# chinhau5/parallel_eda

Hardware: AMD Instinct MI355X
Metric: place+route wall-clock to feasibility (s/flow; bitcoin_miner-scale synthetic on stratixiv-like fabric) (lower is better)
Workload: dtype fp32; 1 GPU; model=bitcoin_miner, arch=bitcoin_stratixiv, grid=280x200, W=300, rr_nodes=15745036, rr_edges=87277236, blocks=37632, nets=35616, conns=110426, global_batch=110426, seq_len=0, final_overused=0, wirelength=4914127

## Files before the change

csrc/hip/place_kernel.hip:

```cpp
#include "pnr_hip.h"

namespace pnrh {

struct PlaceDev {
  const int32_t* net_blk_ptr;
  const int32_t* net_blks;
  const int32_t* blk_net_ptr;
  const int32_t* blk_nets;
  const int8_t* blk_type;
  const int8_t* tile_btype;
  const int32_t* type_cols;
  const int32_t* type_col_ptr;
  const uint8_t* fixed;
  const float* net_q;
  const int32_t* net_sink_ptr;
  const float* conn_crit;
  const float* delay_mat;
  int32_t* bx;
  int32_t* by;
  int32_t* bslot;
  int32_t* grid;
  float* net_cost;
  float* net_tcost;
  int32_t num_blocks, num_nets, gx, gy, cap, nx, ny, io_cap;
  int32_t rx0, rx1;
  const int32_t* macro_of;
  const int32_t* macro_ptr;
  const int32_t* macro_blk;
};

struct MovesDev {
  int32_t* mv_blk;
  int32_t* mv_to;
  int32_t* mv_other;
  float* mv_dbb;
  float* mv_dtd;
  uint8_t* mv_flags;
  int32_t* net_claim;
  int32_t* loc_claim;
  int32_t* counters;
  int32_t n_moves;
};

struct Sched {
  float T; int rlim; float timing_tradeoff, inv_bb_norm, inv_td_norm;
  uint32_t seed, batch;
};

#define PROP_WAVES 4

__device__ __forceinline__ int move_index() {
  return blockIdx.x * PROP_WAVES + (threadIdx.x >> 6);
}

__device__ __forceinline__ uint32_t rng_hash(uint32_t a, uint32_t b, uint32_t c) {
  uint32_t h = a * 0x9E3779B9u ^ b * 0x85EBCA6Bu ^ c * 0xC2B2AE35u;
  h ^= h >> 16; h *= 0x7FEB352Du; h ^= h >> 15; h *= 0x846CA68Bu; h ^= h >> 16;
  return h;
}

__device__ __forceinline__ bool is_io_loc(const PlaceDev& p, int x, int y) {
  return x == 0 || x == p.gx - 1 || y == 0 || y == p.gy - 1;
}
__device__ __forceinline__ int cap_at(const PlaceDev& p, int x, int y) {
  bool io = is_io_loc(p, x, y);
  if (!io && x >= 1 && x <= p.nx && y >= 1 && y <= p.ny) return 1;
  if (io && ((x >= 1 && x <= p.nx) != (y >= 1 && y <= p.ny))) return p.io_cap;
  return 0;
}

struct SwapPos {
  int32_t b1; int x1, y1; int32_t b2; int x2, y2;
  __device__ __forceinline__ void operator()(
      const PlaceDev&, int32_t b, int& x, int& y) const {
    if (b == b1) { x = x1; y = y1; }
    else if (b == b2) { x = x2; y = y2; }
  }
};
struct MacroPos {
  int mid, ddx, ddy;
  __device__ __forceinline__ void operator()(
      const PlaceDev& p, int32_t b, int& x, int& y) const {
    if (p.macro_of[b] == mid) { x += ddx; y += ddy; }
  }
};

template <class Pos> __device__ __forceinline__
float net_bb_cost(const PlaceDev& p, int n, const Pos& pos) {
  int xmin = 1 << 28, xmax = -1, ymin = 1 << 28, ymax = -1;
  int32_t e0 = p.net_blk_ptr[n], e1 = p.net_blk_ptr[n + 1];
  for (int32_t e = e0; e < e1; ++e) {
    int32_t b = p.net_blks[e];
    int x = p.bx[b], y = p.by[b];
    pos(p, b, x, y);
    xmin = min(xmin, x); xmax = max(xmax, x);
    ymin = min(ymin, y); ymax = max(ymax, y);
  }
  return p.net_q[n] * ((xmax - xmin + 1) + (ymax - ymin + 1));
}

template <class Pos> __device__ __forceinline__
float net_td_cost(const PlaceDev& p, int n, const Pos& pos) {
  if (p.delay_mat == nullptr) return 0.0f;
  int32_t e0 = p.net_blk_ptr[n], e1 = p.net_blk_ptr[n + 1];
  int32_t drv = p.net_blks[e0];
  int dx0 = p.bx[drv], dy0 = p.by[drv];
  pos(p, drv, dx0, dy0);
  float t = 0.0f;
  int32_t c0 = p.net_sink_ptr[n];
  for (int32_t e = e0 + 1; e < e1; ++e) {
    int32_t b = p.net_blks[e];
    int x = p.bx[b], y = p.by[b];
    pos(p, b, x, y);
    int dx = abs(x - dx0), dy = abs(y - dy0);
    t += p.conn_crit[c0 + (e - e0 - 1)] * p.delay_mat[dx * p.gy + dy];
  }
  return t;
}

__device__ __forceinline__ float wave_sum_f32(float v) {
  for (int off = 32; off; off >>= 1) v += __shfl_xor(v, off);
  return v;
}

__device__ __forceinline__
bool blk_has_net(const PlaceDev& p, int32_t b, int32_t n) {
  int32_t lo = p.blk_net_ptr[b], hi = p.blk_net_ptr[b + 1];
  while (lo < hi) {
    int32_t mid2 = (lo + hi) >> 1;
    if (p.blk_nets[mid2] < n) lo = mid2 + 1; else hi = mid2;
  }
  return lo < p.blk_net_ptr[b + 1] && p.blk_nets[lo] == n;
}

template <class F> __device__ __forceinline__
void for_blk_nets(const PlaceDev& p, int32_t b, F f) {
  for (int32_t k = p.blk_net_ptr[b] + (threadIdx.x & 63);
       k < p.blk_net_ptr[b + 1]; k += 64)
    f(p.blk_nets[k]);
}
template <class F> __device__ __forceinline__
void for_macro_nets(const PlaceDev& p, int32_t mm0, int32_t mm1, F f) {
  for (int32_t j = mm0; j < mm1; ++j)
    for_blk_nets(p, p.macro_blk[j], [&](int32_t n) { f(j, n); });
}

struct MinClaims {
  int32_t* net; int32_t* loc; int32_t mine;
  __device__ __forceinline__ void take_net(int n) const { atomicMin(&net[n], mine); }
  __device__ __forceinline__ void take_loc(int t) const { atomicMin(&loc[t], mine); }
  __device__ __forceinline__ bool holds_net(int n) const { return net[n] == mine; }
  __device__ __forceinline__ bool holds_loc(int t) const { return loc[t] == mine; }
};
struct EpochClaims {
  unsigned long long* net; unsigned long long* loc; unsigned long long mine;
  __device__ __forceinline__ void take_net(int n) const { atomicMax(&net[n], mine); }
  __device__ __forceinline__ void take_loc(int t) const { atomicMax(&loc[t], mine); }
  __device__ __forceinline__ bool holds_net(int n) const { return net[n] == mine; }
  __device__ __forceinline__ bool holds_loc(int t) const { return loc[t] == mine; }
};

__device__ __forceinline__ unsigned long long claim_key(uint32_t batch, int i) {
  return ((unsigned long long)batch << 32) | (0xFFFFFFFFu - (uint32_t)i);
}

__device__ __forceinline__
int propose_select(const PlaceDev& p, int rlim, uint32_t seed, uint32_t batch,
                   int i, int& x1o, int& y1o, int& slot1o) {
  uint32_t r0 = rng_hash(seed ^ 0x5BD1E995u, batch, i);
  int32_t blk = r0 % p.num_blocks;
  if (p.fixed && p.fixed[blk]) return -1;
  if (p.rx0 >= 0 && (p.bx[blk] < p.rx0 || p.bx[blk] > p.rx1))
    return -1;
  bool io = p.blk_type[blk] == 0;
  int x0 = p.bx[blk], y0 = p.by[blk];
  int x1 = -1, y1 = -1, slot1 = 0;
  int bt = p.blk_type[blk];
  if (p.tile_btype && bt >= 2 && p.type_cols) {
    int c0 = p.type_col_ptr[bt - 2], c1 = p.type_col_ptr[bt - 1];
    int lo = c0, hi = c1;
    while (lo < hi) { int m = (lo + hi) >> 1;
                      if (p.type_cols[m] < x0 - rlim) lo = m + 1; else hi = m; }
    int lo2 = lo, hi2 = c1;
    while (lo2 < hi2) { int m = (lo2 + hi2) >> 1;
                        if (p.type_cols[m] <= x0 + rlim) lo2 = m + 1; else hi2 = m; }
    int ncol = lo2 - lo;
    if (ncol > 0) {
      int ylo = max(1, y0 - rlim), yhi = min(p.ny, y0 + rlim);
      for (int att = 0; att < 8; ++att) {
        uint32_t r1 = rng_hash(seed, batch, i * 131 + 7 * att + 1);
        uint32_t r2 = rng_hash(seed, batch, i * 131 + 7 * att + 2);
        int tx = p.type_cols[lo + (int)(r1 % ncol)];
        if (p.rx0 >= 0 && (tx < p.rx0 || tx > p.rx1)) continue;
        int ty = ylo + (int)(r2 % (yhi - ylo + 1));
        if (tx == x0 && ty == y0) continue;
        x1 = tx; y1 = ty; slot1 = 0;
        break;
      }
    }
  } else {
    for (int att = 0; att < 8; ++att) {
      uint32_t r1 = rng_hash(seed, batch, i * 131 + 7 * att + 1);
      uint32_t r2 = rng_hash(seed, batch, i * 131 + 7 * att + 2);
      int tx = x0 + (int)(r1 % (2 * rlim + 1)) - rlim;
      int ty = y0 + (int)(r2 % (2 * rlim + 1)) - rlim;
      if (tx < 0 || tx >= p.gx || ty < 0 || ty >= p.gy) continue;
      if (p.rx0 >= 0 && (tx < p.rx0 || tx > p.rx1)) continue;
      if (p.tile_btype) {
        if (p.tile_btype[tx * p.gy + ty] != p.blk_type[blk]) continue;
      } else if (is_io_loc(p, tx, ty) != io) continue;
      int c = cap_at(p, tx, ty);
      if (c <= 0) continue;
      if (tx == x0 && ty == y0) continue;
      x1 = tx; y1 = ty;
      slot1 = (int)(rng_hash(seed, batch, i * 131 + 7 * att + 3) % c);
      break;
    }
  }
  if (x1 < 0) return -1;
  x1o = x1; y1o = y1; slot1o = slot1;
  return blk;
}

__device__ __forceinline__
bool macro_shift_ok(const PlaceDev& p, const MacroPos& ms, int32_t mm0,
                    int32_t mm1) {
  for (int32_t j = mm0; j < mm1; ++j) {
    int32_t b = p.macro_blk[j];
    int sx = p.bx[b], sy = p.by[b];
    int tx = sx + ms.ddx, ty = sy + ms.ddy;
    if (p.fixed && p.fixed[b]) return false;
    if (tx < 0 || tx >= p.gx || ty < 0 || ty >= p.gy) return false;
    if (p.rx0 >= 0 && (tx < p.rx0 || tx > p.rx1 ||
                       sx < p.rx0 || sx > p.rx1)) return false;
    if (p.tile_btype
            ? (p.tile_btype[tx * p.gy + ty] != p.blk_type[b])
            : (is_io_loc(p, tx, ty) != (p.blk_type[b] == 0))) return false;
    if (cap_at(p, tx, ty) != 1) return false;
    int32_t occ = p.grid[((int64_t)tx * p.gy + ty) * p.cap];
    if (occ >= 0 && p.macro_of[occ] != ms.mid) return false;
  }
  return true;
}

template <class Pos> __device__ __forceinline__
void add_net_delta(const PlaceDev& p, int32_t n, const Pos& pos,
                   float timing_tradeoff, float& dbb, float& dtd) {
  dbb += net_bb_cost(p, n, pos) - p.net_cost[n];
  if (timing_tradeoff > 0.0f)
    dtd += net_td_cost(p, n, pos) - p.net_tcost[n];
}

__device__ __forceinline__
bool metropolis(const Sched& s, int i, float& dbb, float& dtd) {
  dbb = wave_sum_f32(dbb);
  dtd = wave_sum_f32(dtd);
  float delta = (1.0f - s.timing_tradeoff) * dbb * s.inv_bb_norm +
                s.timing_tradeoff * dtd * s.inv_td_norm;
  if (delta <= 0.0f) return true;
  if (s.T <= 0.0f) return false;
  float u = (rng_hash(s.seed, s.batch, i * 131 + 5) & 0xFFFFFF) *
            (1.0f / 16777216.0f);
  return u < __expf(-delta / s.T);
}

__device__ __forceinline__
void record_move(const MovesDev& m, int32_t* mv_from, int i, int32_t blk,
                 int32_t to, int32_t other, float dbb, float dtd,
                 int32_t from) {
  atomicAdd(&m.counters[1], 1);
  m.mv_blk[i] = blk;
  m.mv_to[i] = to;
  m.mv_other[i] = other;
  m.mv_dbb[i] = dbb;
  m.mv_dtd[i] = dtd;
  m.mv_flags[i] = 1;
  mv_from[i] = from;
}

template <class Claims> __device__ __forceinline__
void propose_move(const PlaceDev& p, const MovesDev& m, const Claims& c,
                  int32_t* mv_from, int i, const Sched& s) {
  const int lane = threadIdx.x & 63;
  int sel = -1, sx1 = -1, sy1 = -1, sslot = 0;
  if (lane == 0) {
    m.mv_flags[i] = 0;
    sel = propose_select(p, s.rlim, s.seed, s.batch, i, sx1, sy1, sslot);
  }
  sel = __shfl(sel, 0);
  if (sel < 0) return;
  const int x1 = __shfl(sx1, 0);
  const int y1 = __shfl(sy1, 0);
  const int slot1 = __shfl(sslot, 0);
  const int32_t blk = sel;
  const int x0 = p.bx[blk], y0 = p.by[blk];
  const int mid = p.macro_of ? p.macro_of[blk] : -1;
  float dbb = 0.0f, dtd = 0.0f;
  if (mid >= 0) {
    const MacroPos ms{mid, x1 - x0, y1 - y0};
    const int32_t mm0 = p.macro_ptr[mid], mm1 = p.macro_ptr[mid + 1];
    if (mm1 - mm0 > 16) return;
    int ok = 0;
    if (lane == 0) {
      ok = macro_shift_ok(p, ms, mm0, mm1);
      if (ok) atomicAdd(&m.counters[0], 1);
    }
    ok = __shfl(ok, 0);
    if (!ok) return;
    for_macro_nets(p, mm0, mm1, [&](int32_t j, int32_t n) {
      bool dup = false;
      for (int32_t j2 = mm0; j2 < j && !dup; ++j2)
        dup = blk_has_net(p, p.macro_blk[j2], n);
      if (!dup) add_net_delta(p, n, ms, s.timing_tradeoff, dbb, dtd);
    });
    if (!metropolis(s, i, dbb, dtd)) return;
    if (lane == 0)
      record_move(m, mv_from, i, blk,
                  ((ms.ddx + 4096) << 13) | (ms.ddy + 4096), -2 - mid, dbb,
                  dtd, x0 * p.gy + y0);
    for_macro_nets(p, mm0, mm1, [&](int32_t, int32_t n) { c.take_net(n); });
    for (int32_t j = mm0 + lane; j < mm1; j += 64) {
      int32_t b = p.macro_blk[j];
      c.take_loc(p.bx[b] * p.gy + p.by[b]);
      c.take_loc((p.bx[b] + ms.ddx) * p.gy + p.by[b] + ms.ddy);
    }
    return;
  }
  int32_t other = p.grid[((int64_t)x1 * p.gy + y1) * p.cap + slot1];
  if (other == blk) return;
  if (other >= 0 && p.fixed && p.fixed[other]) return;
  if (other >= 0 && p.macro_of && p.macro_of[other] >= 0)
    return;
  if (lane == 0) atomicAdd(&m.counters[0], 1);
  const SwapPos sw{blk, x1, y1, other, other >= 0 ? x0 : -1000,
                   other >= 0 ? y0 : -1000};
  for_blk_nets(p, blk, [&](int32_t n) {
    add_net_delta(p, n, sw, s.timing_tradeoff, dbb, dtd);
  });
  if (other >= 0)
    for_blk_nets(p, other, [&](int32_t n) {
      if (!blk_has_net(p, blk, n))
        add_net_delta(p, n, sw, s.timing_tradeoff, dbb, dtd);
    });
  if (!metropolis(s, i, dbb, dtd)) return;
  if (lane == 0) {
    record_move(m, mv_from, i, blk, (x1 * p.gy + y1) * p.cap + slot1, other,
                dbb, dtd, x0 * p.gy + y0);
    c.take_loc(x0 * p.gy + y0);
    c.take_loc(x1 * p.gy + y1);
  }
  auto take = [&](int32_t n) { c.take_net(n); };
  for_blk_nets(p, blk, take);
  if (other >= 0) for_blk_nets(p, other, take);
}

struct Move {
  int32_t blk, other, to;
  __device__ __forceinline__ Move(const MovesDev& m, int i)
      : blk(m.mv_blk[i]), other(m.mv_other[i]), to(m.mv_to[i]) {}
  __device__ __forceinline__ bool is_macro() const { return other <= -2; }
  __device__ __forceinline__ MacroPos macro() const {
    return MacroPos{-2 - other, (to >> 13) - 4096, (to & 0x1FFF) - 4096};
  }
};

template <class Claims> __device__ __forceinline__
bool resolve_move(const PlaceDev& p, const MovesDev& m, const Claims& c,
                  const int32_t* mv_from, int i, const Move& mv) {
  const int lane = threadIdx.x & 63;
  bool bad = false;
  if (mv.is_macro()) {
    const MacroPos ms = mv.macro();
    const int32_t mm0 = p.macro_ptr[ms.mid], mm1 = p.macro_ptr[ms.mid + 1];
    for (int32_t j = mm0 + lane; j < mm1; j += 64) {
      int32_t b = p.macro_blk[j];
      int sx = p.bx[b], sy = p.by[b];
      int tx = sx + ms.ddx, ty = sy + ms.ddy;
      if (tx < 0 || tx >= p.gx || ty < 0 || ty >= p.gy) bad = true;
      else if (!c.holds_loc(sx * p.gy + sy) ||
               !c.holds_loc(tx * p.gy + ty)) bad = true;
    }
    for_macro_nets(p, mm0, mm1, [&](int32_t, int32_t n) {
      if (!c.holds_net(n)) bad = true;
    });
  } else {
    int x1 = mv.to / p.cap / p.gy, y1 = (mv.to / p.cap) % p.gy;
    if (lane == 0 && (!c.holds_loc(mv_from[i]) ||
                      !c.holds_loc(x1 * p.gy + y1))) bad = true;
    auto lost = [&](int32_t n) { if (!c.holds_net(n)) bad = true; };
    for_blk_nets(p, mv.blk, lost);
    if (mv.other >= 0) for_blk_nets(p, mv.other, lost);
  }
  const bool win = !__any(bad);
  if (lane == 0) {
    if (!win) { m.mv_flags[i] = 0; atomicAdd(&m.counters[3], 1); }
    else { m.mv_flags[i] = 2; atomicAdd(&m.counters[2], 1); }
  }
  return win;
}

template <class Pos> __device__ __forceinline__
void refresh_net(const PlaceDev& p, int32_t n, const Pos& pos,
                 float timing_tradeoff) {
  p.net_cost[n] = net_bb_cost(p, n, pos);
  if (timing_tradeoff > 0.0f) p.net_tcost[n] = net_td_cost(p, n, pos);
}

__device__ __forceinline__
void apply_move(const PlaceDev& p, const MovesDev& m, int i, const Move& mv,
                float timing_tradeoff, double* cost_acc ) {
  const int lane = threadIdx.x & 63;
  if (mv.is_macro()) {
    const MacroPos ms = mv.macro();
    const int32_t mm0 = p.macro_ptr[ms.mid], mm1 = p.macro_ptr[ms.mid + 1];
    for_macro_nets(p, mm0, mm1, [&](int32_t, int32_t n) {
      refresh_net(p, n, ms, timing_tradeoff);
    });
    if (lane == 0) {
      for (int32_t j = mm0; j < mm1; ++j) {
        int32_t b = p.macro_blk[j];
        p.grid[((int64_t)p.bx[b] * p.gy + p.by[b]) * p.cap + p.bslot[b]] = -1;
      }
      for (int32_t j = mm0; j < mm1; ++j) {
        int32_t b = p.macro_blk[j];
        int tx = p.bx[b] + ms.ddx, ty = p.by[b] + ms.ddy;
        p.grid[((int64_t)tx * p.gy + ty) * p.cap] = b;
        p.bx[b] = tx; p.by[b] = ty; p.bslot[b] = 0;
      }
    }
  } else {
    const int32_t blk = mv.blk, other = mv.other;
    int slot1 = mv.to % p.cap;
    int x1 = mv.to / p.cap / p.gy, y1 = (mv.to / p.cap) % p.gy;
    int x0 = p.bx[blk], y0 = p.by[blk], s0 = p.bslot[blk];
    const SwapPos sw{blk, x1, y1, other, other >= 0 ? x0 : -1000,
                     other >= 0 ? y0 : -1000};
    auto refresh = [&](int32_t n) { refresh_net(p, n, sw, timing_tradeoff); };
    for_blk_nets(p, blk, refresh);
    if (other >= 0) for_blk_nets(p, other, refresh);
    if (lane == 0) {
      p.grid[((int64_t)x0 * p.gy + y0) * p.cap + s0] = other >= 0 ? other : -1;
      p.grid[((int64_t)x1 * p.gy + y1) * p.cap + slot1] = blk;
      p.bx[blk] = x1; p.by[blk] = y1; p.bslot[blk] = slot1;
      if (other >= 0) { p.bx[other] = x0; p.by[other] = y0; p.bslot[other] = s0; }
    }
  }
  if (lane == 0) {
    unsafeAtomicAdd(&cost_acc[0], (double)m.mv_dbb[i]);
    unsafeAtomicAdd(&cost_acc[1], (double)m.mv_dtd[i]);
  }
}

__global__ void place_reset_claims_kernel(int32_t* net_claim, int32_t nn,
                                          int32_t* loc_claim, int32_t nl) {
  int i = blockIdx.x * blockDim.x + threadIdx.x;
  int total = max(nn, nl);
  for (; i < total; i += gridDim.x * blockDim.x) {
    if (i < nn) net_claim[i] = 0x7FFFFFFF;
    if (i < nl) loc_claim[i] = 0x7FFFFFFF;
  }
}

__launch_bounds__(64 * PROP_WAVES, 2)
__global__ void place_propose_kernel(PlaceDev p, MovesDev m, int32_t* mv_from,
                                     Sched s) {
  const int i = move_index();
  if (i >= m.n_moves) return;
  propose_move(p, m, MinClaims{m.net_claim, m.loc_claim, i}, mv_from, i, s);
}

__launch_bounds__(64 * PROP_WAVES, 2)
__global__ void place_resolve_kernel(PlaceDev p, MovesDev m,
                                     const int32_t* mv_from) {
  const int i = move_index();
  if (i >= m.n_moves || m.mv_flags[i] != 1) return;
  resolve_move(p, m, MinClaims{m.net_claim, m.loc_claim, i}, mv_from, i,
               Move(m, i));
}

__launch_bounds__(64 * PROP_WAVES, 2)
__global__ void place_apply_kernel(PlaceDev p, MovesDev m,
                                   float timing_tradeoff, double* cost_acc) {
  const int i = move_index();
  if (i >= m.n_moves || m.mv_flags[i] != 2) return;
  apply_move(p, m, i, Move(m, i), timing_tradeoff, cost_acc);
}

struct RunDev {
  int32_t* mv_from;
  unsigned long long* net_claim;
  unsigned long long* loc_claim;
  int32_t* ctrl;
};

__launch_bounds__(64 * PROP_WAVES, 2)
__global__ void place_propose_run_kernel(PlaceDev p, MovesDev m, RunDev r,
                                         Sched s) {
  if (r.ctrl[0]) return;
  const int i = move_index();
  if (i >= m.n_moves) return;
  const EpochClaims c{r.net_claim, r.loc_claim, claim_key(s.batch, i)};
  propose_move(p, m, c, r.mv_from, i, s);
}

__device__ __forceinline__
void commit_move(const PlaceDev& p, const MovesDev& m, const RunDev& r,
                 float timing_tradeoff, double* cost_acc, uint32_t batch) {
  const int i = move_index();
  if (i >= m.n_moves || m.mv_flags[i] != 1) return;
  const Move mv(m, i);
  const EpochClaims c{r.net_claim, r.loc_claim, claim_key(batch, i)};
  if (resolve_move(p, m, c, r.mv_from, i, mv))
    apply_move(p, m, i, mv, timing_tradeoff, cost_acc);
}

__launch_bounds__(64 * PROP_WAVES, 2)
__global__ void place_commit_kernel(PlaceDev p, MovesDev m, RunDev r,
                                    float timing_tradeoff, double* cost_acc,
                                    uint32_t batch, int check,
                                    int32_t target_moves) {
  if (r.ctrl[0]) return;
  commit_move(p, m, r, timing_tradeoff, cost_acc, batch);
  if (!check) return;
  asm volatile("s_waitcnt vmcnt(0)" ::: "memory");
  __syncthreads();
  if (threadIdx.x != 0) return;
  __threadfence();
  asm volatile("s_waitcnt vmcnt(0)" ::: "memory");
  int ticket = __hip_atomic_fetch_add(&r.ctrl[2], 1, __ATOMIC_RELAXED,
                                      __HIP_MEMORY_SCOPE_AGENT);
  if (ticket != (int)gridDim.x - 1) return;
  __threadfence();
  int att = __hip_atomic_load(&m.counters[0], __ATOMIC_RELAXED,
                              __HIP_MEMORY_SCOPE_AGENT);
  int acc = __hip_atomic_load(&m.counters[1], __ATOMIC_RELAXED,
                              __HIP_MEMORY_SCOPE_AGENT);
  int win = __hip_atomic_load(&m.counters[2], __ATOMIC_RELAXED,
                              __HIP_MEMORY_SCOPE_AGENT);
  r.ctrl[1] += 4;
  if (win + (att - acc) >= target_moves) r.ctrl[0] = 1;
  __hip_atomic_store(&r.ctrl[2], 0, __ATOMIC_RELAXED,
                     __HIP_MEMORY_SCOPE_AGENT);
}

__global__ void place_refresh_costs_kernel(PlaceDev p, float timing_tradeoff,
                                           double* out ) {
  int n = blockIdx.x * blockDim.x + threadIdx.x;
  for (; n < p.num_nets; n += gridDim.x * blockDim.x) {
    const SwapPos as_is{-1, 0, 0, -1, 0, 0};
    float c = net_bb_cost(p, n, as_is);
    p.net_cost[n] = c;
    unsafeAtomicAdd(&out[0], (double)c);
    float t = timing_tradeoff > 0.0f ? net_td_cost(p, n, as_is) : 0.0f;
    p.net_tcost[n] = t;
    unsafeAtomicAdd(&out[1], (double)t);
  }
}

}

using namespace pnrh;

extern "C" {

struct PlaceLaunchArgs {
  const int32_t* net_blk_ptr; const int32_t* net_blks;
  const int32_t* blk_net_ptr; const int32_t* blk_nets;
  const int8_t* blk_type; const int8_t* tile_btype;
  const int32_t* type_cols; const int32_t* type_col_ptr;
  const uint8_t* fixed;
  const float* net_q;
  const int32_t* net_sink_ptr; const float* conn_crit; const float* delay_mat;
  int32_t* bx; int32_t* by; int32_t* bslot; int32_t* grid;
  float* net_cost; float* net_tcost;
  int32_t num_blocks, num_nets, gx, gy, cap, nx, ny, io_cap;
  int32_t rx0, rx1;
  const int32_t* macro_of; const int32_t* macro_ptr;
  const int32_t* macro_blk;
  int32_t* mv_blk; int32_t* mv_to; int32_t* mv_other;
  float* mv_dbb; float* mv_dtd; uint8_t* mv_flags;
  int32_t* net_claim; int32_t* loc_claim; int32_t* counters;
  int32_t n_moves;
  float T; int32_t rlim; float timing_tradeoff;
  float inv_bb_norm, inv_td_norm;
  uint32_t seed, batch;
  double* cost_acc;
  int32_t* mv_from;
  unsigned long long* net_claim64; unsigned long long* loc_claim64;
  int32_t* run_ctrl;
};

static void unpack(const PlaceLaunchArgs* a, PlaceDev& p, MovesDev& m) {
  p.net_blk_ptr = a->net_blk_ptr; p.net_blks = a->net_blks;
  p.blk_net_ptr = a->blk_net_ptr; p.blk_nets = a->blk_nets;
  p.blk_type = a->blk_type; p.tile_btype = a->tile_btype;
  p.type_cols = a->type_cols; p.type_col_ptr = a->type_col_ptr;
  p.fixed = a->fixed;
  p.net_q = a->net_q;
  p.net_sink_ptr = a->net_sink_ptr; p.conn_crit = a->conn_crit;
  p.delay_mat = a->delay_mat;
  p.bx = a->bx; p.by = a->by; p.bslot = a->bslot; p.grid = a->grid;
  p.net_cost = a->net_cost; p.net_tcost = a->net_tcost;
  p.num_blocks = a->num_blocks; p.num_nets = a->num_nets;
  p.gx = a->gx; p.gy = a->gy; p.cap = a->cap;
  p.nx = a->nx; p.ny = a->ny; p.io_cap = a->io_cap;
  p.rx0 = a->rx0; p.rx1 = a->rx1;
  p.macro_of = a->macro_of; p.macro_ptr = a->macro_ptr;
  p.macro_blk = a->macro_blk;
  m.mv_blk = a->mv_blk; m.mv_to = a->mv_to; m.mv_other = a->mv_other;
  m.mv_dbb = a->mv_dbb; m.mv_dtd = a->mv_dtd; m.mv_flags = a->mv_flags;
  m.net_claim = a->net_claim; m.loc_claim = a->loc_claim;
  m.counters = a->counters; m.n_moves = a->n_moves;
}

static Sched sched(const PlaceLaunchArgs* a, uint32_t batch) {
  return Sched{a->T, a->rlim, a->timing_tradeoff, a->inv_bb_norm,
               a->inv_td_norm, a->seed, batch};
}

int pnr_place_batch(const PlaceLaunchArgs* a, void* stream) {
  if (!a->mv_from || !a->net_claim || !a->loc_claim)
    return (int)hipErrorInvalidValue;
  PlaceDev p; MovesDev m;
  unpack(a, p, m);
  hipStream_t s = (hipStream_t)stream;
  int rg = (max(max(a->num_nets, a->gx * a->gy), a->n_moves) + 255) / 256;
  rg = rg < 2048 ? rg : 2048;
  hipLaunchKernelGGL(place_reset_claims_kernel, dim3(rg), dim3(256), 0, s,
                     m.net_claim, p.num_nets, m.loc_claim, p.gx * p.gy);
  int mg = (m.n_moves + PROP_WAVES - 1) / PROP_WAVES;
  hipLaunchKernelGGL(place_propose_kernel, dim3(mg), dim3(64 * PROP_WAVES),
                     0, s, p, m, a->mv_from, sched(a, a->batch));
  hipLaunchKernelGGL(place_resolve_kernel, dim3(mg), dim3(64 * PROP_WAVES),
                     0, s, p, m, (const int32_t*)a->mv_from);
  hipLaunchKernelGGL(place_apply_kernel, dim3(mg), dim3(64 * PROP_WAVES),
                     0, s, p, m, a->timing_tradeoff, a->cost_acc);
  return (int)hipGetLastError();
}

int pnr_place_run(const PlaceLaunchArgs* a, uint32_t first_batch,
                  int32_t target_moves, int32_t n_batches, void* stream) {
  if (n_batches < 0 || (n_batches & 3) || first_batch == 0 ||
      !a->mv_from || !a->net_claim64 || !a->loc_claim64 || !a->run_ctrl)
    return (int)hipErrorInvalidValue;
  PlaceDev p; MovesDev m;
  unpack(a, p, m);
  RunDev r;
  r.mv_from = a->mv_from;
  r.net_claim = a->net_claim64; r.loc_claim = a->loc_claim64;
  r.ctrl = a->run_ctrl;
  hipStream_t s = (hipStream_t)stream;
  int mg = (m.n_moves + PROP_WAVES - 1) / PROP_WAVES;
  for (int32_t k = 0; k < n_batches; ++k) {
    const uint32_t batch = first_batch + (uint32_t)k;
    hipLaunchKernelGGL(place_propose_run_kernel, dim3(mg),
                       dim3(64 * PROP_WAVES), 0, s, p, m, r, sched(a, batch));
    hipLaunchKernelGGL(place_commit_kernel, dim3(mg), dim3(64 * PROP_WAVES),
                       0, s, p, m, r, a->timing_tradeoff, a->cost_acc, batch,
                       (int)(((k + 1) & 3) == 0), target_moves);
  }
  return (int)hipGetLastError();
}

int pnr_place_refresh(const PlaceLaunchArgs* a, void* stream) {
  PlaceDev p; MovesDev m;
  unpack(a, p, m);
  hipStream_t s = (hipStream_t)stream;
  hipLaunchKernelGGL(place_refresh_costs_kernel, dim3(1024), dim3(256), 0, s,
                     p, a->timing_tradeoff, a->cost_acc);
  return (int)hipGetLastError();
}

int64_t pnr_place_args_sizeof() { return (int64_t)sizeof(PlaceLaunchArgs); }

}
```

parallel_eda_amd/place/gpu_placer.py:

```python
import ctypes as ct
import math

import numpy as np

from ..arch.archdef import ArchDef
from ..ops import hip_api
from .placer import Placement, analytic_delay_matrix


class PlaceLaunchArgs(ct.Structure):
    _fields_ = [
        ("net_blk_ptr", ct.c_void_p), ("net_blks", ct.c_void_p),
        ("blk_net_ptr", ct.c_void_p), ("blk_nets", ct.c_void_p),
        ("blk_type", ct.c_void_p), ("tile_btype", ct.c_void_p),
        ("type_cols", ct.c_void_p), ("type_col_ptr", ct.c_void_p),
        ("fixed", ct.c_void_p),
        ("net_q", ct.c_void_p),
        ("net_sink_ptr", ct.c_void_p), ("conn_crit", ct.c_void_p),
        ("delay_mat", ct.c_void_p),
        ("bx", ct.c_void_p), ("by", ct.c_void_p), ("bslot", ct.c_void_p),
        ("grid", ct.c_void_p),
        ("net_cost", ct.c_void_p), ("net_tcost", ct.c_void_p),
        ("num_blocks", ct.c_int32), ("num_nets", ct.c_int32),
        ("gx", ct.c_int32), ("gy", ct.c_int32), ("cap", ct.c_int32),
        ("nx", ct.c_int32), ("ny", ct.c_int32), ("io_cap", ct.c_int32),
        ("rx0", ct.c_int32), ("rx1", ct.c_int32),
        ("macro_of", ct.c_void_p), ("macro_ptr", ct.c_void_p),
        ("macro_blk", ct.c_void_p),
        ("mv_blk", ct.c_void_p), ("mv_to", ct.c_void_p), ("mv_other", ct.c_void_p),
        ("mv_dbb", ct.c_void_p), ("mv_dtd", ct.c_void_p), ("mv_flags", ct.c_void_p),
        ("net_claim", ct.c_void_p), ("loc_claim", ct.c_void_p),
        ("counters", ct.c_void_p), ("n_moves", ct.c_int32),
        ("T", ct.c_float), ("rlim", ct.c_int32), ("timing_tradeoff", ct.c_float),
        ("inv_bb_norm", ct.c_float), ("inv_td_norm", ct.c_float),
        ("seed", ct.c_uint32), ("batch", ct.c_uint32),
        ("cost_acc", ct.c_void_p),
        ("mv_from", ct.c_void_p),
        ("net_claim64", ct.c_void_p), ("loc_claim64", ct.c_void_p),
        ("run_ctrl", ct.c_void_p),
    ]


RUN_CHUNK_BATCHES = 32


def _lib():
    lib = hip_api.lib()
    if not hasattr(lib, "_place_ready"):
        lib.pnr_place_batch.restype = ct.c_int
        lib.pnr_place_batch.argtypes = [ct.POINTER(PlaceLaunchArgs), ct.c_void_p]
        lib.pnr_place_run.restype = ct.c_int
        lib.pnr_place_run.argtypes = [ct.POINTER(PlaceLaunchArgs), ct.c_uint32,
                                      ct.c_int32, ct.c_int32, ct.c_void_p]
        lib.pnr_place_refresh.restype = ct.c_int
        lib.pnr_place_refresh.argtypes = [ct.POINTER(PlaceLaunchArgs), ct.c_void_p]
        lib.pnr_place_args_sizeof.restype = ct.c_int64
        if lib.pnr_place_args_sizeof() != ct.sizeof(PlaceLaunchArgs):
            raise RuntimeError("PlaceLaunchArgs ABI mismatch")
        lib._place_ready = True
    return lib


def ptr(t):
    return ct.c_void_p(t.data_ptr())


class GpuPlacer:
    def __init__(self, netlist, arch: ArchDef, seed=7, timing=False,
                 device="cuda:0", n_moves=None, fixed=None,
                 delay_matrix="analytic", macros=None, legacy_batches=False):
        import torch
        self.torch = torch
        self.legacy_batches = legacy_batches
        self.device = device
        self.arch = arch
        self.nl = netlist
        self.seed = seed
        self.timing = timing
        nb = netlist.num_blocks
        nn = netlist.num_nets
        gx, gy = arch.nx + 2, arch.ny + 2
        self.gx, self.gy = gx, gy
        self.cap = max(1, arch.io_cap)
        self.batch_counter = 0

        counts = 1 + np.diff(netlist.net_sink_ptr)
        net_blk_ptr = np.r_[0, np.cumsum(counts)].astype(np.int32)
        net_blks = np.empty(net_blk_ptr[-1], dtype=np.int32)
        net_blks[net_blk_ptr[:-1]] = netlist.net_driver
        is_sink = np.ones(len(net_blks), dtype=bool)
        is_sink[net_blk_ptr[:-1]] = False
        net_blks[is_sink] = netlist.net_sinks
        net_of_member = np.repeat(np.arange(nn, dtype=np.int64),
                                  np.diff(net_blk_ptr))
        key = net_blks.astype(np.int64) * nn + net_of_member
        key = np.unique(key)
        mb = (key // nn).astype(np.int32)
        blk_nets = (key % nn).astype(np.int32)
        blk_net_ptr = np.zeros(nb + 1, dtype=np.int32)
        np.add.at(blk_net_ptr, mb + 1, 1)
        blk_net_ptr = np.cumsum(blk_net_ptr, dtype=np.int64).astype(np.int32)
        q = _cross_count_vec(counts).astype(np.float32)

        def up(a, dtype=None):
            t = torch.from_numpy(np.ascontiguousarray(a))
            return t.to(device)

        self.t_net_blk_ptr = up(net_blk_ptr)
        self.t_net_blks = up(net_blks)
        self.t_blk_net_ptr = up(blk_net_ptr)
        self.t_blk_nets = up(blk_nets)
        self.t_blk_type = up(netlist.block_type)
        self.t_tile_btype = (up(arch.tile_btype_grid())
                             if arch.is_heterogeneous() else None)
        self.t_type_cols = self.t_type_col_ptr = None
        if arch.is_heterogeneous():
            ram_cols = [x for x in range(1, arch.nx + 1)
                        if arch.col_block_type(x) == 2]
            dsp_cols = [x for x in range(1, arch.nx + 1)
                        if arch.col_block_type(x) == 3]
            self.t_type_cols = up(np.asarray(ram_cols + dsp_cols,
                                             dtype=np.int32))
            self.t_type_col_ptr = up(np.asarray(
                [0, len(ram_cols), len(ram_cols) + len(dsp_cols)],
                dtype=np.int32))
        self.t_net_q = up(q)
        self._fixed = fixed
        self.t_fixed = None
        if fixed is not None:
            mask = np.zeros(nb, dtype=np.uint8)
            mask[np.asarray(fixed[0], dtype=np.int64)] = 1
            self.t_fixed = up(mask)
        self.t_net_sink_ptr = up(netlist.net_sink_ptr.astype(np.int32))
        self.t_conn_crit = torch.zeros(netlist.num_conns, dtype=torch.float32,
                                       device=device)
        if timing:
            if delay_matrix == "routed":
                from .delay_matrix import routed_delay_matrix
                dm = routed_delay_matrix(arch)
            else:
                dm = analytic_delay_matrix(arch)
            self._dm = dm
            self.t_delay_mat = up(dm.ravel())
        else:
            self._dm = None
            self.t_delay_mat = None

        bx, by, bslot, grid = self._initial_placement(seed)
        self.t_macro_of = self.t_macro_ptr = self.t_macro_blk = None
        self.macros = macros or []
        if self.macros:
            bx, by, bslot, grid = self._legalize_macros(
                bx, by, bslot, grid, self.macros)
            macro_of = np.full(nb, -1, dtype=np.int32)
            mptr = [0]
            mblk = []
            for mi, grp in enumerate(self.macros):
                for (b, dx, dy) in grp:
                    macro_of[b] = mi
                    mblk.append(b)
                mptr.append(len(mblk))
            self.t_macro_of = up(macro_of)
            self.t_macro_ptr = up(np.asarray(mptr, dtype=np.int32))
            self.t_macro_blk = up(np.asarray(mblk, dtype=np.int32))
        self.t_bx = up(bx); self.t_by = up(by); self.t_bslot = up(bslot)
        self.t_grid = up(grid)
        self.t_net_cost = torch.zeros(nn, dtype=torch.float32, device=device)
        self.t_net_tcost = torch.zeros(nn, dtype=torch.float32, device=device)

        self.n_moves = n_moves or int(np.clip(nb // 16, 64, 1 << 16))
        nm = self.n_moves
        self.t_mv_blk = torch.zeros(nm, dtype=torch.int32, device=device)
        self.t_mv_to = torch.zeros(nm, dtype=torch.int32, device=device)
        self.t_mv_other = torch.zeros(nm, dtype=torch.int32, device=device)
        self.t_mv_dbb = torch.zeros(nm, dtype=torch.float32, device=device)
        self.t_mv_dtd = torch.zeros(nm, dtype=torch.float32, device=device)
        self.t_mv_flags = torch.zeros(nm, dtype=torch.uint8, device=device)
        self.t_net_claim = self.t_loc_claim = None
        self.t_net_claim64 = self.t_loc_claim64 = None
        if legacy_batches:
            self.t_net_claim = torch.zeros(nn, dtype=torch.int32, device=device)
            self.t_loc_claim = torch.zeros(gx * gy, dtype=torch.int32,
                                           device=device)
        else:
            self.t_net_claim64 = torch.zeros(nn, dtype=torch.int64,
                                             device=device)
            self.t_loc_claim64 = torch.zeros(gx * gy, dtype=torch.int64,
                                             device=device)
        self.t_mv_from = torch.zeros(nm, dtype=torch.int32, device=device)
        self.t_run_state = torch.zeros(8, dtype=torch.int32, device=device)
        self.t_counters = self.t_run_state[:4]
        self.t_run_ctrl = self.t_run_state[4:]
        self.t_cost_acc = torch.zeros(2, dtype=torch.float64, device=device)

        self.lib = _lib()
        self.bb_cost, self.td_cost = self.refresh_costs()

    def _initial_placement(self, seed):
        arch = self.arch
        nl = self.nl
        rng = np.random.default_rng(seed)
        nb = nl.num_blocks
        bx = np.zeros(nb, dtype=np.int32)
        by = np.zeros(nb, dtype=np.int32)
        bslot = np.zeros(nb, dtype=np.int32)
        if self._fixed is not None:
            bx2, by2, bs2, grid = self._initial_placement_free(rng)
            ids, fx, fy, fs = [np.asarray(a) for a in self._fixed]
            for b, x, y, sl in zip(ids, fx, fy, fs):
                occ = grid[x, y, sl]
                if occ == b:
                    continue
                grid[bx2[b], by2[b], bs2[b]] = occ
                if occ >= 0:
                    bx2[occ], by2[occ], bs2[occ] = bx2[b], by2[b], bs2[b]
                bx2[b], by2[b], bs2[b] = x, y, sl
                grid[x, y, sl] = b
            return bx2, by2, bs2, grid.reshape(-1)
        return self._initial_placement_free(rng, flat=True)

    def _legalize_macros(self, bx, by, bslot, grid, macros):
        arch = self.arch
        g = grid.reshape(self.gx, self.gy, self.cap)
        members = [b for grp in macros for (b, _, _) in grp]
        for b in members:
            g[bx[b], by[b], bslot[b]] = -1
        tb = (arch.tile_btype_grid().reshape(self.gx, self.gy)
              if arch.is_heterogeneous() else None)

        def tile_ok(b, x, y):
            if not (0 <= x < self.gx and 0 <= y < self.gy):
                return False
            bt = int(self.nl.block_type[b])
            if tb is not None:
                if tb[x, y] != bt:
                    return False
            else:
                io = (x == 0 or x == self.gx - 1 or
                      y == 0 or y == self.gy - 1)
                inner = 1 <= x <= arch.nx and 1 <= y <= arch.ny
                if bt == 0 or io or not inner:
                    return False
            return g[x, y, 0] < 0

        for grp in macros:
            placed = False
            for ax in range(1, arch.nx + 1):
                for ay in range(1, arch.ny + 1):
                    if all(tile_ok(b, ax + dx, ay + dy)
                           for (b, dx, dy) in grp):
                        for (b, dx, dy) in grp:
                            bx[b], by[b], bslot[b] = ax + dx, ay + dy, 0
                            g[ax + dx, ay + dy, 0] = b
                        placed = True
                        break
                if placed:
                    break
            if not placed:
                raise ValueError("cannot legalize macro (grid too full)")
        return bx, by, bslot, g.reshape(-1)

    def _initial_placement_free(self, rng, flat=False):
        arch = self.arch
        nl = self.nl
        nb = nl.num_blocks
        bx = np.zeros(nb, dtype=np.int32)
        by = np.zeros(nb, dtype=np.int32)
        bslot = np.zeros(nb, dtype=np.int32)
        grid = np.full((self.gx, self.gy, self.cap), -1, dtype=np.int32)
        ios = np.nonzero(nl.block_type == 0)[0]
        if not arch.is_heterogeneous():
            clbs = np.nonzero(nl.block_type == 1)[0]
            tiles = rng.permutation(arch.nx * arch.ny)[:len(clbs)]
            if len(tiles) < len(clbs):
                raise ValueError("too many CLBs for grid")
            bx[clbs] = tiles // arch.ny + 1
            by[clbs] = tiles % arch.ny + 1
            grid[bx[clbs], by[clbs], 0] = clbs
        else:
            col_t = np.asarray([arch.col_block_type(x)
                                for x in range(1, arch.nx + 1)])
            for t in (1, 2, 3):
                blks = np.nonzero(nl.block_type == t)[0]
                if not len(blks):
                    continue
                cols = np.nonzero(col_t == t)[0]
                cand = (cols[:, None] * arch.ny +
                        np.arange(arch.ny)[None, :]).ravel()
                if len(blks) > len(cand):
                    raise ValueError(f"too many type-{t} blocks for grid")
                tiles = cand[rng.permutation(len(cand))[:len(blks)]]
                bx[blks] = tiles // arch.ny + 1
                by[blks] = tiles % arch.ny + 1
                grid[bx[blks], by[blks], 0] = blks
        io_locs = ([(0, y) for y in range(1, arch.ny + 1)] +
                   [(self.gx - 1, y) for y in range(1, arch.ny + 1)] +
                   [(x, 0) for x in range(1, arch.nx + 1)] +
                   [(x, self.gy - 1) for x in range(1, arch.nx + 1)])
        slots = [(x, y, s) for (x, y) in io_locs for s in range(arch.io_cap)]
        sel = rng.permutation(len(slots))[:len(ios)]
        for b, k in zip(ios, sel):
            x, y, s = slots[k]
            bx[b], by[b], bslot[b] = x, y, s
            grid[x, y, s] = b
        return (bx, by, bslot, grid.reshape(-1)) if flat \
            else (bx, by, bslot, grid)

    def _args(self, T=0.0, rlim=1, tt=0.0, inv_bb=1.0, inv_td=1.0):
        a = PlaceLaunchArgs()
        a.net_blk_ptr = ptr(self.t_net_blk_ptr); a.net_blks = ptr(self.t_net_blks)
        a.blk_net_ptr = ptr(self.t_blk_net_ptr); a.blk_nets = ptr(self.t_blk_nets)
        a.blk_type = ptr(self.t_blk_type)
        a.tile_btype = (ptr(self.t_tile_btype)
                        if self.t_tile_btype is not None else None)
        a.type_cols = (ptr(self.t_type_cols)
                       if self.t_type_cols is not None else None)
        a.type_col_ptr = (ptr(self.t_type_col_ptr)
                          if self.t_type_col_ptr is not None else None)
        a.fixed = ptr(self.t_fixed) if self.t_fixed is not None else None
        a.net_q = ptr(self.t_net_q)
        a.net_sink_ptr = ptr(self.t_net_sink_ptr)
        a.conn_crit = ptr(self.t_conn_crit)
        a.delay_mat = ptr(self.t_delay_mat) if self.t_delay_mat is not None else None
        a.bx = ptr(self.t_bx); a.by = ptr(self.t_by); a.bslot = ptr(self.t_bslot)
        a.grid = ptr(self.t_grid)
        a.net_cost = ptr(self.t_net_cost); a.net_tcost = ptr(self.t_net_tcost)
        a.num_blocks = self.nl.num_blocks; a.num_nets = self.nl.num_nets
        a.gx = self.gx; a.gy = self.gy; a.cap = self.cap
        a.nx = self.arch.nx; a.ny = self.arch.ny; a.io_cap = self.arch.io_cap
        a.rx0, a.rx1 = getattr(self, "move_region", (-1, -1))
        if getattr(self, "t_macro_of", None) is not None:
            a.macro_of = ptr(self.t_macro_of)
            a.macro_ptr = ptr(self.t_macro_ptr)
            a.macro_blk = ptr(self.t_macro_blk)
        else:
            a.macro_of = a.macro_ptr = a.macro_blk = None
        a.mv_blk = ptr(self.t_mv_blk); a.mv_to = ptr(self.t_mv_to)
        a.mv_other = ptr(self.t_mv_other); a.mv_dbb = ptr(self.t_mv_dbb)
        a.mv_dtd = ptr(self.t_mv_dtd); a.mv_flags = ptr(self.t_mv_flags)
        if self.legacy_batches:
            a.net_claim = ptr(self.t_net_claim)
            a.loc_claim = ptr(self.t_loc_claim)
            a.net_claim64 = a.loc_claim64 = None
        else:
            a.net_claim = a.loc_claim = None
            a.net_claim64 = ptr(self.t_net_claim64)
            a.loc_claim64 = ptr(self.t_loc_claim64)
        a.mv_from = ptr(self.t_mv_from)
        a.run_ctrl = ptr(self.t_run_ctrl)
        a.counters = ptr(self.t_counters); a.n_moves = self.n_moves
        a.T = T; a.rlim = max(1, int(rlim)); a.timing_tradeoff = tt
        a.inv_bb_norm = inv_bb; a.inv_td_norm = inv_td
        a.seed = self.seed & 0xFFFFFFFF; a.batch = self.batch_counter
        a.cost_acc = ptr(self.t_cost_acc)
        return a

    def _stream(self):
        return self.torch.cuda.current_stream().cuda_stream

    def refresh_costs(self):
        self.t_cost_acc.zero_()
        a = self._args(tt=1.0 if self.timing else 0.0)
        rc = self.lib.pnr_place_refresh(ct.byref(a), self._stream())
        hip_api.check(rc, "place_refresh")
        self.torch.cuda.synchronize(self.device)
        bb, td = self.t_cost_acc.cpu().numpy()
        self.bb_cost, self.td_cost = float(bb), float(td)
        return self.bb_cost, self.td_cost

    def run_batches(self, T, rlim, target_moves, tt, bb_norm, td_norm,
                    max_batches=256):
        if self.legacy_batches:
            return self._run_batches_legacy(T, rlim, target_moves, tt,
                                            bb_norm, td_norm, max_batches)
        self.t_run_state.zero_()
        a = self._args(T=T, rlim=rlim, tt=tt,
                       inv_bb=1.0 / bb_norm, inv_td=1.0 / td_norm)
        target = int(min(max(math.ceil(target_moves), -0x7FFFFFFF),
                         0x7FFFFFFF))
        cap = 4 * ((max_batches + 3) // 4)
        first = self.batch_counter + 1
        enq = 0
        att = acc = executed = 0
        while enq < cap:
            n = min(RUN_CHUNK_BATCHES, cap - enq)
            rc = self.lib.pnr_place_run(ct.byref(a), first + enq, target, n,
                                        self._stream())
            hip_api.check(rc, "place_run")
            enq += n
            st = self.t_run_state.cpu().numpy()
            att, acc = int(st[0]), int(st[1])
            done, executed = int(st[4]), int(st[5])
            if done:
                break
        self.batch_counter += executed
        srate = acc / max(1, att)
        return srate, att

    def _run_batches_legacy(self, T, rlim, target_moves, tt, bb_norm, td_norm,
                            max_batches=256):
        self.t_counters.zero_()
        batches = 0
        win = att = acc = 0
        while batches < max_batches:
            for _ in range(4):
                self.batch_counter += 1
                a = self._args(T=T, rlim=rlim, tt=tt,
                               inv_bb=1.0 / bb_norm, inv_td=1.0 / td_norm)
                rc = self.lib.pnr_place_batch(ct.byref(a), self._stream())
                hip_api.check(rc, "place_batch")
                batches += 1
            self.torch.cuda.synchronize(self.device)
            c = self.t_counters.cpu().numpy()
            att, acc, win = int(c[0]), int(c[1]), int(c[2])
            if win + (att - acc) >= target_moves:
                break
        else:
            self.torch.cuda.synchronize(self.device)
        srate = acc / max(1, att)
        return srate, att

    def set_move_region(self, x0, x1):
        self.move_region = (x0, x1)

    def set_crit(self, conn_crit):
        t = self.torch.from_numpy(np.ascontiguousarray(conn_crit,
                                                       dtype=np.float32))
        self.t_conn_crit.copy_(t.to(self.device))

    def placement(self):
        return Placement(self.t_bx.cpu().numpy(), self.t_by.cpu().numpy(),
                         self.t_bslot.cpu().numpy(),
# ... 160 lines not shown
```

Baseline: 7.846 s.

## Evaluate swap-move net costs in parallel across wave lanes and cache them for commit

```diff
diff --git a/csrc/hip/place_kernel.hip b/csrc/hip/place_kernel.hip
--- a/csrc/hip/place_kernel.hip
+++ b/csrc/hip/place_kernel.hip
@@ -39,8 +39,14 @@
   int32_t* net_claim;
   int32_t* loc_claim;
   int32_t* counters;
+  float* mv_ncost;
+  float* mv_ntcost;
+  int32_t cost_k;
   int32_t n_moves;
 };
+
+#define MV_RECOMPUTE (1 << 30)
+#define COST_NONE (-1.0f)
 
 struct Sched {
   float T; int rlim; float timing_tradeoff, inv_bb_norm, inv_td_norm;
@@ -85,8 +91,13 @@
   }
 };
 
+__device__ __forceinline__ float mul_rn(float a, float b) {
+#pragma clang fp contract(off)
+  return a * b;
+}
+
 template <class Pos> __device__ __forceinline__
-float net_bb_cost(const PlaceDev& p, int n, const Pos& pos) {
+int net_span(const PlaceDev& p, int n, const Pos& pos) {
   int xmin = 1 << 28, xmax = -1, ymin = 1 << 28, ymax = -1;
   int32_t e0 = p.net_blk_ptr[n], e1 = p.net_blk_ptr[n + 1];
   for (int32_t e = e0; e < e1; ++e) {
@@ -96,7 +107,12 @@
     xmin = min(xmin, x); xmax = max(xmax, x);
     ymin = min(ymin, y); ymax = max(ymax, y);
   }
-  return p.net_q[n] * ((xmax - xmin + 1) + (ymax - ymin + 1));
+  return (xmax - xmin + 1) + (ymax - ymin + 1);
+}
+
+template <class Pos> __device__ __forceinline__
+float net_bb_cost(const PlaceDev& p, int n, const Pos& pos) {
+  return mul_rn(p.net_q[n], (float)net_span(p, n, pos));
 }
 
 template <class Pos> __device__ __forceinline__
@@ -113,7 +129,8 @@
     int x = p.bx[b], y = p.by[b];
     pos(p, b, x, y);
     int dx = abs(x - dx0), dy = abs(y - dy0);
-    t += p.conn_crit[c0 + (e - e0 - 1)] * p.delay_mat[dx * p.gy + dy];
+    t = __builtin_fmaf(p.conn_crit[c0 + (e - e0 - 1)],
+                       p.delay_mat[dx * p.gy + dy], t);
   }
   return t;
 }
@@ -134,10 +151,14 @@
 }
 
 template <class F> __device__ __forceinline__
+void for_blk_nets_k(const PlaceDev& p, int32_t b, F f) {
+  const int32_t k0 = p.blk_net_ptr[b];
+  for (int32_t k = k0 + (threadIdx.x & 63); k < p.blk_net_ptr[b + 1]; k += 64)
+    f(k - k0, p.blk_nets[k]);
+}
+template <class F> __device__ __forceinline__
 void for_blk_nets(const PlaceDev& p, int32_t b, F f) {
-  for (int32_t k = p.blk_net_ptr[b] + (threadIdx.x & 63);
-       k < p.blk_net_ptr[b + 1]; k += 64)
-    f(p.blk_nets[k]);
+  for_blk_nets_k(p, b, [&](int32_t, int32_t n) { f(n); });
 }
 template <class F> __device__ __forceinline__
 void for_macro_nets(const PlaceDev& p, int32_t mm0, int32_t mm1, F f) {
@@ -243,20 +264,153 @@
   return true;
 }
 
+struct NetCosts { float bb, td; };
+
 template <class Pos> __device__ __forceinline__
-void add_net_delta(const PlaceDev& p, int32_t n, const Pos& pos,
-                   float timing_tradeoff, float& dbb, float& dtd) {
-  dbb += net_bb_cost(p, n, pos) - p.net_cost[n];
-  if (timing_tradeoff > 0.0f)
-    dtd += net_td_cost(p, n, pos) - p.net_tcost[n];
+NetCosts add_net_delta(const PlaceDev& p, int32_t n, const Pos& pos,
+                       float timing_tradeoff, float& dbb, float& dtd) {
+  const float q = p.net_q[n], span = (float)net_span(p, n, pos);
+  NetCosts c{mul_rn(q, span), 0.0f};
+  dbb += __builtin_fmaf(q, span, -p.net_cost[n]);
+  if (timing_tradeoff > 0.0f) {
+    c.td = net_td_cost(p, n, pos);
+    dtd += c.td - p.net_tcost[n];
+  }
+  return c;
+}
+
+#define EVAL_SLOTS 64
+#define EVAL_ITEMS 256
+struct EvalStage {
+  int32_t incl[EVAL_SLOTS];
+  int32_t e0[EVAL_SLOTS];
+  int32_t c0[EVAL_SLOTS];
+  int32_t drvx[EVAL_SLOTS], drvy[EVAL_SLOTS];
+  int32_t xmin[EVAL_SLOTS], xmax[EVAL_SLOTS];
+  int32_t ymin[EVAL_SLOTS], ymax[EVAL_SLOTS];
+  float crit[EVAL_ITEMS], delay[EVAL_ITEMS];
+};
+
+__device__ __forceinline__ void wave_lds_sync() {
+  __builtin_amdgcn_fence(__ATOMIC_RELEASE, "wavefront");
+  __builtin_amdgcn_wave_barrier();
+  __builtin_amdgcn_fence(__ATOMIC_ACQUIRE, "wavefront");
+}
+
+__device__ __forceinline__
+bool eval_move_parallel(const PlaceDev& p, EvalStage& st, const SwapPos& sw,
+                        int32_t blk, int32_t other, int n_a, int n_b,
+                        bool timing, float& dbb, float& dtd, NetCosts& ca,
+                        NetCosts& cb) {
+  const int lane = threadIdx.x & 63;
+  const int ns = n_a + n_b;
+  int32_t n = -1;
+  if (lane < n_a) n = p.blk_nets[p.blk_net_ptr[blk] + lane];
+  else if (lane < ns) n = p.blk_nets[p.blk_net_ptr[other] + lane - n_a];
+  int lo = 0, hi = n_a;
+  for (int it = 0; it < 7; ++it) {
+    const int mid = (lo + hi) >> 1;
+    const int32_t v = __shfl(n, mid & 63);
+    if (lo < hi) { if (v < n) lo = mid + 1; else hi = mid; }
+  }
+  const int32_t found = __shfl(n, lo & 63);
+  const bool shared = lane >= n_a && lo < n_a && found == n;
+  const bool live = lane < ns && !shared;
+  int32_t e0 = 0, cnt = 0, c0 = 0;
+  int dx0 = 0, dy0 = 0;
+  float q = 0.0f, old_bb = 0.0f, old_td = 0.0f;
+  if (live) {
+    e0 = p.net_blk_ptr[n];
+    cnt = p.net_blk_ptr[n + 1] - e0;
+    q = p.net_q[n];
+    old_bb = p.net_cost[n];
+    if (timing) {
+      old_td = p.net_tcost[n];
+      c0 = p.net_sink_ptr[n];
+      const int32_t drv = p.net_blks[e0];
+      dx0 = p.bx[drv]; dy0 = p.by[drv];
+      sw(p, drv, dx0, dy0);
+    }
+  }
+  int incl = cnt;
+  for (int off = 1; off < 64; off <<= 1) {
+    const int v = __shfl_up(incl, off);
+    if (lane >= off) incl += v;
+  }
+  const int total = __shfl(incl, 63);
+  if (total > EVAL_ITEMS) return false;
+  st.incl[lane] = incl; st.e0[lane] = e0; st.c0[lane] = c0;
+  st.drvx[lane] = dx0; st.drvy[lane] = dy0;
+  st.xmin[lane] = 1 << 28; st.xmax[lane] = -1;
+  st.ymin[lane] = 1 << 28; st.ymax[lane] = -1;
+  wave_lds_sync();
+  for (int base = 0; base < total; base += 64) {
+    const int g = base + lane;
+    if (g >= total) continue;
+    int s0 = 0, s1 = ns - 1;
+    for (int it = 0; it < 6; ++it) {
+      const int mid = (s0 + s1) >> 1;
+      const bool in_low = st.incl[mid] > g;
+      if (s0 < s1) { if (in_low) s1 = mid; else s0 = mid + 1; }
+    }
+    const int slot = s0;
+    const int mbr = g - (slot ? st.incl[slot - 1] : 0);
+    const int32_t b = p.net_blks[st.e0[slot] + mbr];
+    int x = p.bx[b], y = p.by[b];
+    sw(p, b, x, y);
+    atomicMin(&st.xmin[slot], x); atomicMax(&st.xmax[slot], x);
+    atomicMin(&st.ymin[slot], y); atomicMax(&st.ymax[slot], y);
+    if (timing && mbr > 0) {
+      const int dx = abs(x - st.drvx[slot]), dy = abs(y - st.drvy[slot]);
+      st.crit[g] = p.conn_crit[st.c0[slot] + mbr - 1];
+      st.delay[g] = p.delay_mat[dx * p.gy + dy];
+    }
+  }
+  wave_lds_sync();
+  NetCosts nc{COST_NONE, 0.0f};
+  float d_bb = 0.0f, d_td = 0.0f;
+  if (live) {
+    const float span = (float)((st.xmax[lane] - st.xmin[lane] + 1) +
+                               (st.ymax[lane] - st.ymin[lane] + 1));
+    nc.bb = mul_rn(q, span);
+    d_bb = __builtin_fmaf(q, span, -old_bb);
+    if (timing) {
+      float t = 0.0f;
+      const int i0 = incl - cnt;
+      for (int j = 1; j < cnt; ++j)
+        t = __builtin_fmaf(st.crit[i0 + j], st.delay[i0 + j], t);
+      nc.td = t;
+      d_td = t - old_td;
+    }
+  }
+  const int sb = (n_a + lane) & 63;
+  const float b_dbb = __shfl(d_bb, sb), b_dtd = __shfl(d_td, sb);
+  const float b_bb = __shfl(nc.bb, sb), b_td = __shfl(nc.td, sb);
+  if (lane < n_a) {
+    dbb += d_bb;
+    if (timing) dtd += d_td;
+    ca = nc;
+  }
+  if (lane < n_b) {
+    if (b_bb != COST_NONE) {
+      dbb += b_dbb;
+      if (timing) dtd += b_dtd;
+    }
+    cb = NetCosts{b_bb, b_td};
+  }
+  return true;
 }
 
 __device__ __forceinline__
 bool metropolis(const Sched& s, int i, float& dbb, float& dtd) {
   dbb = wave_sum_f32(dbb);
   dtd = wave_sum_f32(dtd);
-  float delta = (1.0f - s.timing_tradeoff) * dbb * s.inv_bb_norm +
-                s.timing_tradeoff * dtd * s.inv_td_norm;
+  float delta;
+  {
+#pragma clang fp contract(off)
+    delta = (1.0f - s.timing_tradeoff) * dbb * s.inv_bb_norm +
+            s.timing_tradeoff * dtd * s.inv_td_norm;
+  }
   if (delta <= 0.0f) return true;
   if (s.T <= 0.0f) return false;
   float u = (rng_hash(s.seed, s.batch, i * 131 + 5) & 0xFFFFFF) *
@@ -334,18 +488,44 @@
   if (lane == 0) atomicAdd(&m.counters[0], 1);
   const SwapPos sw{blk, x1, y1, other, other >= 0 ? x0 : -1000,
                    other >= 0 ? y0 : -1000};
-  for_blk_nets(p, blk, [&](int32_t n) {
-    add_net_delta(p, n, sw, s.timing_tradeoff, dbb, dtd);
-  });
-  if (other >= 0)
-    for_blk_nets(p, other, [&](int32_t n) {
-      if (!blk_has_net(p, blk, n))
-        add_net_delta(p, n, sw, s.timing_tradeoff, dbb, dtd);
+  const int n_a = p.blk_net_ptr[blk + 1] - p.blk_net_ptr[blk];
+  const int n_b =
+      other >= 0 ? p.blk_net_ptr[other + 1] - p.blk_net_ptr[other] : 0;
+  NetCosts ca{COST_NONE, 0.0f}, cb{COST_NONE, 0.0f};
+  __shared__ EvalStage stage[PROP_WAVES];
+  const bool timing = s.timing_tradeoff > 0.0f;
+  bool evaluated = false;
+  if (n_a + n_b <= EVAL_SLOTS && (!timing || p.delay_mat != nullptr))
+    evaluated = eval_move_parallel(p, stage[threadIdx.x >> 6], sw, blk, other,
+                                   n_a, n_b, timing, dbb, dtd, ca, cb);
+  if (!evaluated) {
+    for_blk_nets_k(p, blk, [&](int32_t k, int32_t n) {
+      NetCosts nc = add_net_delta(p, n, sw, s.timing_tradeoff, dbb, dtd);
+      if (k < 64) ca = nc;
     });
+    if (other >= 0)
+      for_blk_nets_k(p, other, [&](int32_t k, int32_t n) {
+        if (blk_has_net(p, blk, n)) return;
+        NetCosts nc = add_net_delta(p, n, sw, s.timing_tradeoff, dbb, dtd);
+        if (k < 64) cb = nc;
+      });
+  }
   if (!metropolis(s, i, dbb, dtd)) return;
+  const bool stored = n_a + n_b <= m.cost_k;
+  if (stored) {
+    const int64_t s0 = (int64_t)i * m.cost_k;
+    if (lane < n_a) m.mv_ncost[s0 + lane] = ca.bb;
+    if (lane < n_b) m.mv_ncost[s0 + n_a + lane] = cb.bb;
+    if (s.timing_tradeoff > 0.0f) {
+      if (lane < n_a) m.mv_ntcost[s0 + lane] = ca.td;
+      if (lane < n_b) m.mv_ntcost[s0 + n_a + lane] = cb.td;
+    }
+  }
   if (lane == 0) {
-    record_move(m, mv_from, i, blk, (x1 * p.gy + y1) * p.cap + slot1, other,
-                dbb, dtd, x0 * p.gy + y0);
+    record_move(m, mv_from, i, blk,
+                ((x1 * p.gy + y1) * p.cap + slot1) |
+                    (stored ? 0 : MV_RECOMPUTE),
+                other, dbb, dtd, x0 * p.gy + y0);
     c.take_loc(x0 * p.gy + y0);
     c.take_loc(x1 * p.gy + y1);
   }
@@ -356,8 +536,12 @@
 
 struct Move {
   int32_t blk, other, to;
+  bool recompute;
   __device__ __forceinline__ Move(const MovesDev& m, int i)
-      : blk(m.mv_blk[i]), other(m.mv_other[i]), to(m.mv_to[i]) {}
+      : blk(m.mv_blk[i]), other(m.mv_other[i]), to(m.mv_to[i]) {
+    recompute = !is_macro() && (to & MV_RECOMPUTE);
+    if (recompute) to &= ~MV_RECOMPUTE;
+  }
   __device__ __forceinline__ bool is_macro() const { return other <= -2; }
   __device__ __forceinline__ MacroPos macro() const {
     return MacroPos{-2 - other, (to >> 13) - 4096, (to & 0x1FFF) - 4096};
@@ -435,9 +619,24 @@
     int x0 = p.bx[blk], y0 = p.by[blk], s0 = p.bslot[blk];
     const SwapPos sw{blk, x1, y1, other, other >= 0 ? x0 : -1000,
                      other >= 0 ? y0 : -1000};
-    auto refresh = [&](int32_t n) { refresh_net(p, n, sw, timing_tradeoff); };
-    for_blk_nets(p, blk, refresh);
-    if (other >= 0) for_blk_nets(p, other, refresh);
+    if (mv.recompute) {
+      auto refresh = [&](int32_t n) { refresh_net(p, n, sw, timing_tradeoff); };
+      for_blk_nets(p, blk, refresh);
+      if (other >= 0) for_blk_nets(p, other, refresh);
+    } else {
+      const int64_t s0 = (int64_t)i * m.cost_k;
+      int32_t slot0 = 0;
+      auto copy = [&](int32_t k, int32_t n) {
+        const float bb = m.mv_ncost[s0 + slot0 + k];
+        if (bb == COST_NONE) return;
+        p.net_cost[n] = bb;
+        if (timing_tradeoff > 0.0f)
+          p.net_tcost[n] = m.mv_ntcost[s0 + slot0 + k];
+      };
+      for_blk_nets_k(p, blk, copy);
+      slot0 = p.blk_net_ptr[blk + 1] - p.blk_net_ptr[blk];
+      if (other >= 0) for_blk_nets_k(p, other, copy);
+    }
     if (lane == 0) {
       p.grid[((int64_t)x0 * p.gy + y0) * p.cap + s0] = other >= 0 ? other : -1;
       p.grid[((int64_t)x1 * p.gy + y1) * p.cap + slot1] = blk;
@@ -588,6 +787,8 @@
   int32_t* mv_from;
   unsigned long long* net_claim64; unsigned long long* loc_claim64;
   int32_t* run_ctrl;
+  float* mv_ncost; float* mv_ntcost;
+  int32_t cost_k;
 };
 
 static void unpack(const PlaceLaunchArgs* a, PlaceDev& p, MovesDev& m) {
@@ -611,6 +812,14 @@
   m.mv_dbb = a->mv_dbb; m.mv_dtd = a->mv_dtd; m.mv_flags = a->mv_flags;
   m.net_claim = a->net_claim; m.loc_claim = a->loc_claim;
   m.counters = a->counters; m.n_moves = a->n_moves;
+  m.mv_ncost = a->mv_ncost; m.mv_ntcost = a->mv_ntcost;
+  m.cost_k = a->cost_k;
+}
+
+static bool batch_args_ok(const PlaceLaunchArgs* a) {
+  return a->mv_from && a->mv_ncost && a->mv_ntcost && a->cost_k >= 1 &&
+         a->cost_k <= 64 &&
+         (int64_t)a->gx * a->gy * a->cap < (int64_t)MV_RECOMPUTE;
 }
 
 static Sched sched(const PlaceLaunchArgs* a, uint32_t batch) {
@@ -619,7 +828,7 @@
 }
 
 int pnr_place_batch(const PlaceLaunchArgs* a, void* stream) {
-  if (!a->mv_from || !a->net_claim || !a->loc_claim)
+  if (!batch_args_ok(a) || !a->net_claim || !a->loc_claim)
     return (int)hipErrorInvalidValue;
   PlaceDev p; MovesDev m;
   unpack(a, p, m);
@@ -641,7 +850,8 @@
 int pnr_place_run(const PlaceLaunchArgs* a, uint32_t first_batch,
                   int32_t target_moves, int32_t n_batches, void* stream) {
   if (n_batches < 0 || (n_batches & 3) || first_batch == 0 ||
-      !a->mv_from || !a->net_claim64 || !a->loc_claim64 || !a->run_ctrl)
+      !batch_args_ok(a) || !a->net_claim64 || !a->loc_claim64 ||
+      !a->run_ctrl)
     return (int)hipErrorInvalidValue;
   PlaceDev p; MovesDev m;
   unpack(a, p, m);
diff --git a/parallel_eda_amd/place/gpu_placer.py b/parallel_eda_amd/place/gpu_placer.py
--- a/parallel_eda_amd/place/gpu_placer.py
+++ b/parallel_eda_amd/place/gpu_placer.py
@@ -38,6 +38,8 @@
         ("mv_from", ct.c_void_p),
         ("net_claim64", ct.c_void_p), ("loc_claim64", ct.c_void_p),
         ("run_ctrl", ct.c_void_p),
+        ("mv_ncost", ct.c_void_p), ("mv_ntcost", ct.c_void_p),
+        ("cost_k", ct.c_int32),
     ]
 
 
@@ -188,6 +190,12 @@
             self.t_loc_claim64 = torch.zeros(gx * gy, dtype=torch.int64,
                                              device=device)
         self.t_mv_from = torch.zeros(nm, dtype=torch.int32, device=device)
+        max_deg = int(np.diff(blk_net_ptr).max()) if nb else 0
+        self.cost_k = int(np.clip(2 * max_deg, 1, 64))
+        self.t_mv_ncost = torch.zeros(nm * self.cost_k, dtype=torch.float32,
+                                      device=device)
+        self.t_mv_ntcost = torch.zeros(nm * self.cost_k, dtype=torch.float32,
+                                       device=device)
         self.t_run_state = torch.zeros(8, dtype=torch.int32, device=device)
         self.t_counters = self.t_run_state[:4]
         self.t_run_ctrl = self.t_run_state[4:]
@@ -348,6 +356,8 @@
             a.loc_claim64 = ptr(self.t_loc_claim64)
         a.mv_from = ptr(self.t_mv_from)
         a.run_ctrl = ptr(self.t_run_ctrl)
+        a.mv_ncost = ptr(self.t_mv_ncost); a.mv_ntcost = ptr(self.t_mv_ntcost)
+        a.cost_k = self.cost_k
         a.counters = ptr(self.t_counters); a.n_moves = self.n_moves
         a.T = T; a.rlim = max(1, int(rlim)); a.timing_tradeoff = tt
         a.inv_bb_norm = inv_bb; a.inv_td_norm = inv_td
```

Result: faster. 7.124 s (median of 6 runs) (-9.2%).
